# Project-MONAI/GenerativeModels

Measured on NVIDIA H100. Metric: ddim50_voxels_per_s, higher is better.
Workload: dtype fp16

## Files before the change

generativemodels_b200/csrc/flash_attn.cu:

```cuda
#include "common.cuh"
#include "wgmma.cuh"
#include <cuda.h>
#include <cudaTypedefs.h>
#include <mutex>
#include <string.h>

namespace b200 {

struct FlashDev {
  alignas(64) CUtensorMap tmQ;
  alignas(64) CUtensorMap tmK;
  alignas(64) CUtensorMap tmVt;
  int B, T, S, heads, dh, d_chunks;
  int q_tiles, q_tiles_grid, n_items, n_kv;
  float scale_log2;
  h16* out;
  long long out_bstride, out_pitch;
  const h16* res;
  long long res_bstride, res_pitch;
};

namespace fa {

static constexpr int kThreads = 128;
static constexpr int kBM = 64, kBKV = 64;
static constexpr int kChunkBytes = 64 * 64 * 2;

__device__ __forceinline__ uint32_t smem_u32(const void* p) {
  return static_cast<uint32_t>(__cvta_generic_to_shared(p));
}
__device__ __forceinline__ void mbar_init(uint32_t bar, uint32_t count) {
  asm volatile("mbarrier.init.shared::cta.b64 [%0], %1;" ::"r"(bar), "r"(count));
}
__device__ __forceinline__ void mbar_expect_tx(uint32_t bar, uint32_t bytes) {
  asm volatile("mbarrier.arrive.expect_tx.shared::cta.b64 _, [%0], %1;" ::"r"(bar), "r"(bytes) : "memory");
}
__device__ __forceinline__ void mbar_wait(uint32_t bar, uint32_t parity) {
  uint32_t done;
  do {
    asm volatile(
        "{\n\t.reg .pred p;\n\t"
        "mbarrier.try_wait.parity.shared::cta.b64 p, [%1], %2;\n\t"
        "selp.u32 %0, 1, 0, p;\n\t}"
        : "=r"(done)
        : "r"(bar), "r"(parity)
        : "memory");
  } while (!done);
}
__device__ __forceinline__ void mbar_arrive_cluster(uint32_t bar, uint32_t cta) {
  uint32_t remote;
  asm volatile("mapa.shared::cluster.u32 %0, %1, %2;" : "=r"(remote) : "r"(bar), "r"(cta));
  asm volatile("mbarrier.arrive.shared::cluster.b64 _, [%0];" ::"r"(remote) : "memory");
}
__device__ __forceinline__ void tma_load_3d(const CUtensorMap* tm, uint32_t bar, uint32_t dst, int c0, int c1, int c2) {
  asm volatile(
      "cp.async.bulk.tensor.3d.shared::cluster.global.mbarrier::complete_tx::bytes"
      " [%0], [%1, {%3, %4, %5}], [%2];" ::"r"(dst),
      "l"(reinterpret_cast<uint64_t>(tm)), "r"(bar), "r"(c0), "r"(c1), "r"(c2)
      : "memory");
}
__device__ __forceinline__ void tma_load_3d_multicast(const CUtensorMap* tm, uint32_t bar, uint32_t dst, int c0, int c1,
                                                      int c2, uint16_t cta_mask) {
  asm volatile(
      "cp.async.bulk.tensor.3d.shared::cluster.global.mbarrier::complete_tx::bytes.multicast::cluster"
      " [%0], [%1, {%3, %4, %5}], [%2], %6;" ::"r"(dst),
      "l"(reinterpret_cast<uint64_t>(tm)), "r"(bar), "r"(c0), "r"(c1), "r"(c2), "h"(cta_mask)
      : "memory");
}
__device__ __forceinline__ uint32_t cluster_ctarank() {
  uint32_t r;
  asm volatile("mov.u32 %0, %%cluster_ctarank;" : "=r"(r));
  return r;
}
__device__ __forceinline__ void cluster_sync() {
  asm volatile("barrier.cluster.arrive.release.aligned;\n\tbarrier.cluster.wait.acquire.aligned;" ::: "memory");
}
__device__ __forceinline__ void named_sync(uint32_t id, uint32_t threads) {
  asm volatile("bar.sync %0, %1;" ::"r"(id), "r"(threads) : "memory");
}
__device__ __forceinline__ float ex2_approx(float x) {
  float y;
  asm("ex2.approx.ftz.f32 %0, %1;" : "=f"(y) : "f"(x));
  return y;
}
__device__ __forceinline__ uint32_t pack_h2(float lo, float hi) {
  h162 v = f2h2(lo, hi);
  return *reinterpret_cast<uint32_t*>(&v);
}

template <int DCH>
__global__ void __launch_bounds__(kThreads, 1) flash_attn_kernel(const __grid_constant__ FlashDev p) {
  constexpr int DV = 64 * DCH;
  extern __shared__ uint8_t smem_raw[];
  const uint32_t q_base = (smem_u32(smem_raw) + 1023u) & ~1023u;
// ... 11 lines not shown
  const int q0 = qt * kBM;
  const int qc = h * p.dh;
  const int vc = qc;

  pdl_launch_dependents();
  if (tid == 0) {
    mbar_init(q_bar, 1);
    mbar_init(k_bar, 1);
    mbar_init(v_bar, 1);
    asm volatile("fence.mbarrier_init.release.cluster;" ::: "memory");
    asm volatile("fence.proxy.async.shared::cta;" ::: "memory");
  }
  __syncthreads();
  pdl_wait();
  if (tid == 0) {
    mbar_expect_tx(q_bar, DCH * kChunkBytes);
    for (int c = 0; c < DCH; ++c) tma_load_3d(&p.tmQ, q_bar, q_base + c * kChunkBytes, qc + 64 * c, q0, b);
    mbar_expect_tx(k_bar, DCH * kChunkBytes);
    for (int c = 0; c < DCH; ++c) tma_load_3d(&p.tmK, k_bar, k_base + c * kChunkBytes, qc + 64 * c, 0, b);
    mbar_expect_tx(v_bar, DV * kBKV * 2);
    tma_load_3d(&p.tmVt, v_bar, v_base, 0, vc, b);
  }

  float o[DV / 2];
#pragma unroll
  for (int i = 0; i < DV / 2; ++i) o[i] = 0.f;
  float m0 = -INFINITY, m1 = -INFINITY, l0 = 0.f, l1 = 0.f;
  const float sc = p.scale_log2;
  mbar_wait(q_bar, 0);

  for (int j = 0; j < p.n_kv; ++j) {
    const uint32_t ph = j & 1;
    float s[32];
    mbar_wait(k_bar, ph);
    wgmma_fence();
#pragma unroll
    for (int c = 0; c < DCH; ++c) {
      const uint64_t qd = wgmma_desc(q_base + c * kChunkBytes), kd = wgmma_desc(k_base + c * kChunkBytes);
#pragma unroll
      for (int kk = 0; kk < 4; ++kk) wgmma_ss<64>(s, qd + 2u * kk, kd + 2u * kk, (c | kk) != 0 ? 1u : 0u);
    }
    wgmma_commit();
    wgmma_wait<0>();
    wgmma_touch<32>(s);
    __syncthreads();
    if (tid == 0 && j + 1 < p.n_kv) {
      mbar_expect_tx(k_bar, DCH * kChunkBytes);
      for (int c = 0; c < DCH; ++c) tma_load_3d(&p.tmK, k_bar, k_base + c * kChunkBytes, qc + 64 * c, (j + 1) * kBKV, b);
    }

    const int key0 = j * kBKV + 2 * (lane & 3);
    float mx0 = -INFINITY, mx1 = -INFINITY;
#pragma unroll
    for (int n = 0; n < 8; ++n) {
#pragma unroll
      for (int e = 0; e < 2; ++e) {
        const bool ok = key0 + 8 * n + e < p.S;
        s[4 * n + e] = ok ? s[4 * n + e] * sc : -INFINITY;
        s[4 * n + 2 + e] = ok ? s[4 * n + 2 + e] * sc : -INFINITY;
        mx0 = fmaxf(mx0, s[4 * n + e]);
        mx1 = fmaxf(mx1, s[4 * n + 2 + e]);
      }
// ... 24 lines not shown
    for (int n = 0; n < DV / 8; ++n) {
      o[4 * n] *= a0; o[4 * n + 1] *= a0;
      o[4 * n + 2] *= a1; o[4 * n + 3] *= a1;
    }

    mbar_wait(v_bar, ph);
    wgmma_fence();
    const uint64_t vd = wgmma_desc(v_base);
#pragma unroll
    for (int kk = 0; kk < 4; ++kk) wgmma_rs<DV>(o, pa + 4 * kk, vd + 2u * kk, 1u);
    wgmma_commit();
    wgmma_wait<0>();
    wgmma_touch<DV / 2>(o);
    __syncthreads();
    if (tid == 0 && j + 1 < p.n_kv) {
      mbar_expect_tx(v_bar, DV * kBKV * 2);
      tma_load_3d(&p.tmVt, v_bar, v_base, (j + 1) * kBKV, vc, b);
    }
  }

  l0 += __shfl_xor_sync(0xffffffffu, l0, 1);
  l0 += __shfl_xor_sync(0xffffffffu, l0, 2);
  l1 += __shfl_xor_sync(0xffffffffu, l1, 1);
  l1 += __shfl_xor_sync(0xffffffffu, l1, 2);
  const float inv0 = 1.f / l0, inv1 = 1.f / l1;
  const int r0 = 16 * warp + (lane >> 2);
#pragma unroll
  for (int half = 0; half < 2; ++half) {
    const int t = q0 + r0 + 8 * half;
    if (t >= p.T) continue;
    const float inv = half ? inv1 : inv0;
// ... 56 lines not shown
  pdl_launch_dependents();
  if (tid == 0) {
    mbar_init(q_bar, 1);
    for (int s = 0; s < kRing; ++s) {
      mbar_init(full0 + 8 * s, 1);
      mbar_init(empty0 + 8 * s, 4 * kCluster);
    }
    asm volatile("fence.mbarrier_init.release.cluster;" ::: "memory");
  }
  cluster_sync();
  pdl_wait();

  if (wg == 0) {
    setmaxnreg_dec<kProducerRegs>();
    if (tid == 0) {
      mbar_expect_tx(q_bar, 8 * kChunkBytes);
      for (int c = 0; c < 8; ++c) tma_load_3d(&p.tmQ, q_bar, q_base + c * kChunkBytes, qc + 64 * c, q0, b);
      for (int j = 0; j < p.n_kv; ++j) {
        for (int n = 0; n < kChunksPerBlock; ++n) {
          const int slot = n % kRing;
          mbar_wait(empty0 + 8 * slot, ((n / kRing) & 1) ^ 1);
          mbar_expect_tx(full0 + 8 * slot, kChunkBytes);
          if ((n & 1) != (int)rank) continue;
          const uint32_t dst = ring + slot * kChunkBytes, fb = full0 + 8 * slot;
          if (n < 16) {
            const int d = (n & 3) | ((n >> 3) << 2);
            tma_load_3d_multicast(&p.tmK, fb, dst, qc + 64 * d, j * kBlockKeys + 64 * ((n >> 2) & 1), b, 0x3);
          } else {
            const int g = (n - 16) >> 2;
            tma_load_3d_multicast(&p.tmVt, fb, dst, j * kBlockKeys + 64 * (g >> 1), qc + 256 * (g & 1) + 64 * (n & 3), b,
                                  0x3);
          }
        }
      }
    }
  } else {
    setmaxnreg_inc<kConsumerRegs>();
// ... 268 lines not shown
```

generativemodels_b200/csrc/igemm.cu:

```cuda
#include "common.cuh"
#include "wgmma.cuh"
#include <cuda.h>
#include <cudaTypedefs.h>
#include <mutex>
#include <stdlib.h>
#include <string.h>

namespace b200 {

static constexpr int kBM = 128;
static constexpr int kBK = 64;
static constexpr int kABytes = kBM * kBK * 2;
static constexpr int kMmaWarp0 = 4;
static constexpr int kTmaWarp = 12;
static constexpr int kThreads = 13 * 32;

struct SegDev {
  int8_t src, dw, dh, dd;
  uint16_t c0, nchunks;
};

struct IgemmDev {
  alignas(64) CUtensorMap tmA[2];
  alignas(64) CUtensorMap tmB;
// ... 26 lines not shown
  long long out_sN, out_sD, out_sH, out_sW;
  const float* bias;
  const float* rowvec;
  long long rowvec_bstride;
  const float* row_bias;
  int act1, act2;
  int bias_prefetch;
  int geglu;
  float scale;
  const void* res_ptr;
  int res_dtype, res_vec, res_v256;
  long long res_sN, res_sD, res_sH, res_sW;
  SegDev seg[B200_IGEMM_MAX_SEG];
};

__device__ __forceinline__ uint32_t smem_u32(const void* p) {
  return static_cast<uint32_t>(__cvta_generic_to_shared(p));
}
__device__ __forceinline__ void mbar_init(uint32_t bar, uint32_t count) {
  asm volatile("mbarrier.init.shared::cta.b64 [%0], %1;" ::"r"(bar), "r"(count));
}
__device__ __forceinline__ void mbar_arrive_expect_tx(uint32_t bar, uint32_t bytes) {
  asm volatile("mbarrier.arrive.expect_tx.shared::cta.b64 _, [%0], %1;" ::"r"(bar), "r"(bytes) : "memory");
}
__device__ __forceinline__ void mbar_arrive(uint32_t bar) {
  asm volatile("mbarrier.arrive.shared::cta.b64 _, [%0];" ::"r"(bar) : "memory");
}
__device__ __forceinline__ void mbar_wait(uint32_t bar, uint32_t parity) {
  uint32_t done;
  do {
    asm volatile(
        "{\n\t.reg .pred p;\n\t"
        "mbarrier.try_wait.parity.shared::cta.b64 p, [%1], %2;\n\t"
        "selp.u32 %0, 1, 0, p;\n\t}"
        : "=r"(done)
        : "r"(bar), "r"(parity)
        : "memory");
  } while (!done);
}
__device__ __forceinline__ void mbar_wait_warp(uint32_t bar, uint32_t parity) {
  if ((threadIdx.x & 31) == 0) mbar_wait(bar, parity);
  __syncwarp();
}
__device__ __forceinline__ void tma_load_5d(const CUtensorMap* tm, uint32_t bar, uint32_t dst, int c0,
                                            int c1, int c2, int c3, int c4) {
  asm volatile(
      "cp.async.bulk.tensor.5d.shared::cluster.global.mbarrier::complete_tx::bytes"
      " [%0], [%1, {%3, %4, %5, %6, %7}], [%2];" ::"r"(dst),
      "l"(reinterpret_cast<uint64_t>(tm)), "r"(bar), "r"(c0), "r"(c1), "r"(c2), "r"(c3), "r"(c4)
      : "memory");
}
__device__ __forceinline__ void tma_load_3d(const CUtensorMap* tm, uint32_t bar, uint32_t dst, int c0,
                                            int c1, int c2) {
  asm volatile(
      "cp.async.bulk.tensor.3d.shared::cluster.global.mbarrier::complete_tx::bytes"
      " [%0], [%1, {%3, %4, %5}], [%2];" ::"r"(dst),
      "l"(reinterpret_cast<uint64_t>(tm)), "r"(bar), "r"(c0), "r"(c1), "r"(c2)
      : "memory");
}
template <int CH>
__device__ __forceinline__ void acc_ld(const float* src, uint32_t* r) {
#pragma unroll
  for (int j = 0; j < CH; j += 4) {
    const float4 t = *reinterpret_cast<const float4*>(src + j);
    r[j] = __float_as_uint(t.x); r[j + 1] = __float_as_uint(t.y);
    r[j + 2] = __float_as_uint(t.z); r[j + 3] = __float_as_uint(t.w);
  }
}

__host__ __device__ __forceinline__ int split_begin(int num_k, int splits, int ks) {
  return (int)(((long long)num_k * ks) / splits);
}

template <int CH>
// ... 153 lines not shown
    }
  }
  act_inplace<CH>(v, p.act2);
  if (p.out_dtype == B200_DT_H16) {
    h16* o = reinterpret_cast<h16*>(p.out_ptr) + out_off + col0;
    uint4 pk[CH / 8];
#pragma unroll
    for (int g = 0; g < CH / 8; ++g) pk[g] = pack8(v + g * 8);
    if (p.out_v256) {
#pragma unroll
      for (int g = 0; g < CH / 16; ++g) stg256(o + g * 16, pk[2 * g], pk[2 * g + 1]);
    } else {
#pragma unroll
      for (int g = 0; g < CH / 8; ++g) *reinterpret_cast<uint4*>(o + g * 8) = pk[g];
    }
    if constexpr (CH == 32) {
      if (gs) {
        if (p.gn_sh == 3) {
#pragma unroll
          for (int g = 0; g < 4; ++g) {
            float f[8];
            unpack8(pk[g], f);
#pragma unroll
            for (int j = 0; j < 8; ++j) { gs[g] += f[j]; gs[4 + g] = fmaf(f[j], f[j], gs[4 + g]); }
          }
        } else {
#pragma unroll
          for (int g = 0; g < 4; ++g) {
            float f[8];
            unpack8(pk[g], f);
#pragma unroll
            for (int j = 0; j < 8; ++j) {
              gs[2 * g + (j >> 2)] += f[j];
              gs[8 + 2 * g + (j >> 2)] = fmaf(f[j], f[j], gs[8 + 2 * g + (j >> 2)]);
            }
          }
        }
      }
    }
  } else {
    float* o = reinterpret_cast<float*>(p.out_ptr) + out_off + col0;
#pragma unroll
    for (int g = 0; g < CH / 4; ++g)
      *reinterpret_cast<float4*>(o + g * 4) = make_float4(v[g * 4], v[g * 4 + 1], v[g * 4 + 2], v[g * 4 + 3]);
  }
}

template <int CH>
__device__ __forceinline__ void epilogue_row(const IgemmDev& p, float* v, int nb, int ow, long long out_off,
                                             long long res_off, int col0) {
// ... 540 lines not shown
      if (want_key >= 0) {
#pragma unroll
        for (int i = 0; i < PER; ++i)
          if (lane + 32 * i < BN) addv_other[lane + 32 * i] = nbv[i] + nrw[i];
        next_key = want_key;
      }
      __syncwarp();
      if (lane == 0) mbar_arrive(tempty_bar);
    }
    if (gn_on) { __syncwarp(); gn_flush(); }
  }

  __syncthreads();
}

__global__ void igemm_check_kernel(const __grid_constant__ IgemmDev p) {
  pdl_entry();
  const long long rows = (long long)p.N * p.OD * p.OH * p.OW;
  const int col_groups = (p.out_cols + 15) / 16;
  const long long idx = (long long)blockIdx.x * blockDim.x + threadIdx.x;
  if (idx >= rows * col_groups) return;
  const int cg = (int)(idx % col_groups);
  long long m = idx / col_groups;
  const int ow = (int)(m % p.OW); m /= p.OW;
  const int oh = (int)(m % p.OH); m /= p.OH;
  const int od = (int)(m % p.OD); m /= p.OD;
  const int nb = (int)m;
  float acc[16];
#pragma unroll
  for (int j = 0; j < 16; ++j) acc[j] = 0.f;
// ... 145 lines not shown
    v[0] += a.x; v[1] += a.y; v[2] += a.z; v[3] += a.w;
    v[4] += b.x; v[5] += b.y; v[6] += b.z; v[7] += b.w;
  }
  const long long out_off = nb * p.out_sN + od * p.out_sD + oh * p.out_sH + ow * p.out_sW;
  const long long res_off = nb * p.res_sN + od * p.res_sD + oh * p.res_sH + ow * p.res_sW;
  epilogue_math<8>(p, v, nb, ow, res_off, col0);
  store_direct<8>(p, v, out_off, col0);
}

struct Plan {
  TileShape ts;
  long long m_tiles, ntiles, rows;
  int kchunks, BN, tiles_n;
  int splits, ws_cols;
  long long ws_bytes;
};
static int env_int(const char* name, int dflt) {
  const char* e = getenv(name);
  return (e && *e) ? atoi(e) : dflt;
}
static int narrow_min_chunks() { static int v = env_int("B200_NARROW_MIN_CHUNKS", 4); return v; }
static int bias_prefetch_mode() { static int v = env_int("B200_BIAS_PREFETCH", 1); return v; }
static int no_v256() { static int v = env_int("B200_NO_V256", 0); return v; }
static int narrow_one_wave() { static int v = env_int("B200_NARROW_ONE_WAVE", 1); return v; }
static int split_min() { static int v = env_int("B200_SPLIT_MIN", 3); return v; }
static int split_range_min() { static int v = env_int("B200_SPLIT_RANGE_MIN", 32); return v < 1 ? 1 : v; }
static Plan make_plan(const b200_igemm_params* p, bool allow_split, int nsm = 0) {
  if (nsm <= 0) nsm = sm_count();
  Plan pl;
  pl.kchunks = 0;
  for (int s = 0; s < p->n_seg; ++s) pl.kchunks += p->seg[s].nchunks;
  pl.ts = choose_tile(p->out_W, p->out_H, p->out_D, p->stride_w, p->stride_h, p->stride_d);
  const long long tw = (p->out_W + pl.ts.bw - 1) / pl.ts.bw, th = (p->out_H + pl.ts.bh - 1) / pl.ts.bh,
                  td = (p->out_D + pl.ts.bd - 1) / pl.ts.bd;
  pl.m_tiles = tw * th * td * p->out_N;
  pl.rows = (long long)p->out_N * p->out_D * p->out_H * p->out_W;
  pl.splits = 1;
  pl.ws_cols = ((p->out_cols + 7) / 8) * 8;
  pl.ws_bytes = 0;
  const int cols16 = (((p->act1 == B200_ACT_GEGLU ? p->cout : p->out_cols) + 15) / 16) * 16;
  int BN = cols16 <= 16 ? 16 : cols16 <= 32 ? 32 : cols16 <= 64 ? 64 : 128;
  if (p->stat_ptr) BN = 128;
  const long long wide_tiles = pl.m_tiles * ((cols16 + BN - 1) / BN);
  if (allow_split && !p->stat_ptr && !p->gn_partial && p->impl != 1 && p->act1 != B200_ACT_GEGLU && pl.kchunks >= 16 &&
      wide_tiles * 2 <= nsm) {
    long long s = nsm / wide_tiles;
    if (s > pl.kchunks / split_range_min()) s = pl.kchunks / split_range_min();
    if (s > 32) s = 32;
    if (s >= split_min()) {
      pl.splits = (int)s;
      pl.ws_bytes = s * pl.rows * pl.ws_cols * 4;
    }
  }
  if (pl.splits == 1) {
// ... 16 lines not shown
  constexpr int kStageBytes = kABytes + BN * kBK * 2;
  constexpr int smem = 1024 + STAGES * kStageBytes + kBM * (BN + 4) * 4 + 256 + 4 * 32 * 33 * 4 + 8 * BN * 4;
  static_assert(smem <= 227 * 1024, "igemm: shared memory over the 227 KB a block may use");
  static std::once_flag attr_once;
  static cudaError_t attr_rc = cudaSuccess;
  std::call_once(attr_once, [] {
    attr_rc = cudaFuncSetAttribute(igemm_tc_kernel<BN, STAGES>, cudaFuncAttributeMaxDynamicSharedMemorySize, smem);
  });
  B200_CUDA(attr_rc);
  const int grid = d.num_tiles < sm_count() ? d.num_tiles : sm_count();
  B200_CUDA(b200::launch_pdl(igemm_tc_kernel<BN, STAGES>, grid, kThreads, smem, stream, d));
  B200_LAUNCH_CHECK("igemm_tc_kernel");
  return B200_OK;
}

static int env_impl() {
  static int v = -1;
  if (v < 0) {
    const char* e = getenv("B200_IGEMM_IMPL");
    v = (e && strcmp(e, "check") == 0) ? 1 : 0;
  }
  return v;
}

}

using namespace b200;

extern "C" int64_t b200_igemm_split_workspace_bytes(const b200_igemm_params* p) {
  if (!p || p->n_seg < 1 || p->n_seg > B200_IGEMM_MAX_SEG || p->out_N < 1 || p->out_D < 1 || p->out_H < 1 ||
      p->out_W < 1 || p->out_cols < 1 || p->stride_d < 1 || p->stride_h < 1 || p->stride_w < 1)
    return 0;
  if ((p->impl ? p->impl : env_impl()) == 1) return 0;
  return make_plan(p, true).ws_bytes;
}

extern "C" int b200_igemm_plan(const b200_igemm_params* p, int32_t sm_count_, int32_t with_workspace, int32_t out[4]) {
// ... 98 lines not shown
  d.stat_ptr = p->stat_ptr;
  if (p->stat_ptr)
    B200_CHECK_ARG(p->out_N == 1 && p->out_D == 1 && p->out_H == 1, "igemm: stat_ptr needs a GEMM-shaped call");
  if (p->res_ptr) {
    const int g = (p->res_dtype == B200_DT_H16) ? 8 : 4;
    d.res_vec = (p->out_cols % g == 0) && (p->res_sN % g == 0) && (p->res_sD % g == 0) &&
                (p->res_sH % g == 0) && (p->res_sW % g == 0) && (((uintptr_t)p->res_ptr) % 16 == 0);
    d.res_v256 = d.res_vec && p->res_dtype == B200_DT_H16 && (p->out_cols % 16 == 0) && (p->res_sN % 16 == 0) &&
                 (p->res_sD % 16 == 0) && (p->res_sH % 16 == 0) && (p->res_sW % 16 == 0) &&
                 (((uintptr_t)p->res_ptr) % 32 == 0);
    B200_CHECK_ARG(!p->gn_partial || (d.res_vec && p->res_dtype == B200_DT_H16),
                   "igemm: gn_partial needs a vector-aligned h16 residual");
  }

  const int impl = p->impl ? p->impl : env_impl();
  if (impl == 1) {
    const long long rows = (long long)d.N * d.OD * d.OH * d.OW;
    const long long total = rows * ((d.out_cols + 15) / 16);
    const int threads = 128;
    const long long blocks = (total + threads - 1) / threads;
    B200_CHECK_ARG(blocks < (1ll << 31), "igemm(check): problem too large");
    B200_CUDA(b200::launch_pdl(igemm_check_kernel, (unsigned)blocks, threads, 0, stream, d));
    B200_LAUNCH_CHECK("igemm_check_kernel");
    if (d.gn_partial) {
      const long long tot = rows * (d.cout >> d.gn_sh);
      B200_CUDA(b200::launch_pdl(gn8_partial_check_kernel, (unsigned)((tot + 255) / 256), 256, 0, stream, d));
      B200_LAUNCH_CHECK("gn8_partial_check_kernel");
    }
    return B200_OK;
  }
// ... 34 lines not shown
                          CU_TENSOR_MAP_SWIZZLE_128B, CU_TENSOR_MAP_L2_PROMOTION_L2_256B,
                          CU_TENSOR_MAP_FLOAT_OOB_FILL_NONE);
    if (r != CUDA_SUCCESS) {
      set_error("igemm: cuTensorMapEncodeTiled(A%d) failed with %d (C=%d pitch=%d in=%dx%dx%dx%d box=%ux%ux%u)",
                s, (int)r, p->a_C[s], p->a_pitch[s], p->in_N, p->in_D, p->in_H, p->in_W, box[1], box[2], box[3]);
      return B200_ECUDA;
    }
  }
  if (!p->a_ptr[1]) d.tmA[1] = d.tmA[0];
  {
    const int wbn = p->w_batched ? p->in_N : 1;
    cuuint64_t dims[3] = {(cuuint64_t)w_K, (cuuint64_t)p->w_rows, (cuuint64_t)wbn};
    cuuint64_t bs = p->w_bstride ? (cuuint64_t)p->w_bstride * 2 : (cuuint64_t)p->w_rows * p->w_pitch * 2;
    cuuint64_t strides[2] = {(cuuint64_t)p->w_pitch * 2, bs};
    B200_CHECK_ARG(bs % 16 == 0, "igemm: weight batch stride not 16-byte aligned");
    cuuint32_t box[3] = {(cuuint32_t)kBK, (cuuint32_t)BN, 1};
    cuuint32_t estr[3] = {1, 1, 1};
    CUresult r = g_encode(&d.tmB, B200_H16_TMAP, 3, const_cast<void*>(p->w_ptr), dims,
                          strides, box, estr, CU_TENSOR_MAP_INTERLEAVE_NONE, CU_TENSOR_MAP_SWIZZLE_128B,
                          CU_TENSOR_MAP_L2_PROMOTION_L2_256B, CU_TENSOR_MAP_FLOAT_OOB_FILL_NONE);
    if (r != CUDA_SUCCESS) {
      set_error("igemm: cuTensorMapEncodeTiled(W) failed with %d (K=%d rows=%d pitch=%d)", (int)r, w_K,
                p->w_rows, p->w_pitch);
      return B200_ECUDA;
    }
  }

  auto launch = [&](const IgemmDev& dev) {
    switch (BN) {
      case 16:  return launch_tc<16, 8>(dev, stream);
      case 32:  return launch_tc<32, 8>(dev, stream);
      case 64:  return launch_tc<64, 6>(dev, stream);
      default:  return launch_tc<128, 4>(dev, stream);
    }
  };
  if (splits == 1) return launch(d);

  if (p->split_counters) {
    B200_CHECK_ARG(pl.ntiles <= B200_IGEMM_SPLIT_COUNTERS, "igemm: %lld output tiles exceed the %d split-K tickets",
                   pl.ntiles, B200_IGEMM_SPLIT_COUNTERS);
    IgemmDev df = d;
    df.k_splits = splits;
// ... 30 lines not shown
```

generativemodels_b200/csrc/wgmma.cuh:

```cuda
#pragma once
#include "common.cuh"

#ifdef B200_H16_IS_BF16
#define B200_WGMMA_AB "bf16"
#else
#define B200_WGMMA_AB "f16"
#endif

namespace b200 {

__device__ __forceinline__ uint64_t wgmma_desc(uint32_t smem_addr) {
  uint64_t d = 0;
  d |= static_cast<uint64_t>((smem_addr & 0x3FFFFu) >> 4);
  d |= static_cast<uint64_t>(1) << 16;
  d |= static_cast<uint64_t>(1024 >> 4) << 32;
  d |= static_cast<uint64_t>(1) << 62;
  return d;
}
__device__ __forceinline__ void wgmma_fence() { asm volatile("wgmma.fence.sync.aligned;" ::: "memory"); }
__device__ __forceinline__ void wgmma_commit() { asm volatile("wgmma.commit_group.sync.aligned;" ::: "memory"); }
template <int N>
__device__ __forceinline__ void wgmma_wait() { asm volatile("wgmma.wait_group.sync.aligned %0;" ::"n"(N) : "memory"); }
template <int R>
__device__ __forceinline__ void wgmma_touch(float* d) {
// ... 96 lines not shown
      "{\n\t.reg .pred p;\n\t"
      "setp.ne.b32 p, %133, 0;\n\t"
      "wgmma.mma_async.sync.aligned.m64n256k16.f32." B200_WGMMA_AB "." B200_WGMMA_AB " "
      "{%0, %1, %2, %3, %4, %5, %6, %7, %8, %9, %10, %11, %12, %13, %14, %15, %16, %17, %18, %19, %20, %21, %22, %23, %24, %25, %26, %27, %28, %29, %30, %31, %32, %33, %34, %35, %36, %37, %38, %39, %40, %41, %42, %43, %44, %45, %46, %47, %48, %49, %50, %51, %52, %53, %54, %55, %56, %57, %58, %59, %60, %61, %62, %63, %64, %65, %66, %67, %68, %69, %70, %71, %72, %73, %74, %75, %76, %77, %78, %79, %80, %81, %82, %83, %84, %85, %86, %87, %88, %89, %90, %91, %92, %93, %94, %95, %96, %97, %98, %99, %100, %101, %102, %103, %104, %105, %106, %107, %108, %109, %110, %111, %112, %113, %114, %115, %116, %117, %118, %119, %120, %121, %122, %123, %124, %125, %126, %127}, {%128, %129, %130, %131}, %132, p, 1, 1, 0;\n\t}"
      : "+f"(d[0]), "+f"(d[1]), "+f"(d[2]), "+f"(d[3]), "+f"(d[4]), "+f"(d[5]), "+f"(d[6]), "+f"(d[7]), "+f"(d[8]), "+f"(d[9]), "+f"(d[10]), "+f"(d[11]), "+f"(d[12]), "+f"(d[13]), "+f"(d[14]), "+f"(d[15]), "+f"(d[16]), "+f"(d[17]), "+f"(d[18]), "+f"(d[19]), "+f"(d[20]), "+f"(d[21]), "+f"(d[22]), "+f"(d[23]), "+f"(d[24]), "+f"(d[25]), "+f"(d[26]), "+f"(d[27]), "+f"(d[28]), "+f"(d[29]), "+f"(d[30]), "+f"(d[31]), "+f"(d[32]), "+f"(d[33]), "+f"(d[34]), "+f"(d[35]), "+f"(d[36]), "+f"(d[37]), "+f"(d[38]), "+f"(d[39]), "+f"(d[40]), "+f"(d[41]), "+f"(d[42]), "+f"(d[43]), "+f"(d[44]), "+f"(d[45]), "+f"(d[46]), "+f"(d[47]), "+f"(d[48]), "+f"(d[49]), "+f"(d[50]), "+f"(d[51]), "+f"(d[52]), "+f"(d[53]), "+f"(d[54]), "+f"(d[55]), "+f"(d[56]), "+f"(d[57]), "+f"(d[58]), "+f"(d[59]), "+f"(d[60]), "+f"(d[61]), "+f"(d[62]), "+f"(d[63]), "+f"(d[64]), "+f"(d[65]), "+f"(d[66]), "+f"(d[67]), "+f"(d[68]), "+f"(d[69]), "+f"(d[70]), "+f"(d[71]), "+f"(d[72]), "+f"(d[73]), "+f"(d[74]), "+f"(d[75]), "+f"(d[76]), "+f"(d[77]), "+f"(d[78]), "+f"(d[79]), "+f"(d[80]), "+f"(d[81]), "+f"(d[82]), "+f"(d[83]), "+f"(d[84]), "+f"(d[85]), "+f"(d[86]), "+f"(d[87]), "+f"(d[88]), "+f"(d[89]), "+f"(d[90]), "+f"(d[91]), "+f"(d[92]), "+f"(d[93]), "+f"(d[94]), "+f"(d[95]), "+f"(d[96]), "+f"(d[97]), "+f"(d[98]), "+f"(d[99]), "+f"(d[100]), "+f"(d[101]), "+f"(d[102]), "+f"(d[103]), "+f"(d[104]), "+f"(d[105]), "+f"(d[106]), "+f"(d[107]), "+f"(d[108]), "+f"(d[109]), "+f"(d[110]), "+f"(d[111]), "+f"(d[112]), "+f"(d[113]), "+f"(d[114]), "+f"(d[115]), "+f"(d[116]), "+f"(d[117]), "+f"(d[118]), "+f"(d[119]), "+f"(d[120]), "+f"(d[121]), "+f"(d[122]), "+f"(d[123]), "+f"(d[124]), "+f"(d[125]), "+f"(d[126]), "+f"(d[127])
      : "r"(a[0]), "r"(a[1]), "r"(a[2]), "r"(a[3]), "l"(bdesc), "r"(accumulate));
}

template <int N>
__device__ __forceinline__ void wgmma_rs(float* d, const uint32_t* a, uint64_t bdesc, uint32_t accumulate) {
  if constexpr (N == 64) wgmma_rs_n64(d, a, bdesc, accumulate);
  else if constexpr (N == 128) wgmma_rs_n128(d, a, bdesc, accumulate);
  else wgmma_rs_n256(d, a, bdesc, accumulate);
}

}
```

Before: 87530.

## Add 2-CTA cluster 128x256 warp-specialized implicit GEMM with multicast weight tiles

Adds a new implicit-GEMM kernel for wide convolutions. It uses 256-column output tiles, a 2-CTA cluster that multicasts weight halves through TMA, a 4-stage mbarrier ring, and one producer warpgroup feeding two consumer warpgroups. The fused epilogue covers bias, residual and group-norm partial statistics. The kernel is picked automatically for large multi-segment convolutions whose cout is a multiple of 256. It aims to raise operand reuse and tensor-core utilisation, at the cost of register pressure, cluster scheduling constraints and a more complex epilogue. Shared mbarrier/TMA helpers move into a common header and the group-norm accumulation is generalised to any CH.

```diff
diff --git a/generativemodels_b200/csrc/flash_attn.cu b/generativemodels_b200/csrc/flash_attn.cu
--- a/generativemodels_b200/csrc/flash_attn.cu
+++ b/generativemodels_b200/csrc/flash_attn.cu
@@ -26,58 +26,6 @@
 static constexpr int kBM = 64, kBKV = 64;
 static constexpr int kChunkBytes = 64 * 64 * 2;
 
-__device__ __forceinline__ uint32_t smem_u32(const void* p) {
-  return static_cast<uint32_t>(__cvta_generic_to_shared(p));
-}
-__device__ __forceinline__ void mbar_init(uint32_t bar, uint32_t count) {
-  asm volatile("mbarrier.init.shared::cta.b64 [%0], %1;" ::"r"(bar), "r"(count));
-}
-__device__ __forceinline__ void mbar_expect_tx(uint32_t bar, uint32_t bytes) {
-  asm volatile("mbarrier.arrive.expect_tx.shared::cta.b64 _, [%0], %1;" ::"r"(bar), "r"(bytes) : "memory");
-}
-__device__ __forceinline__ void mbar_wait(uint32_t bar, uint32_t parity) {
-  uint32_t done;
-  do {
-    asm volatile(
-        "{\n\t.reg .pred p;\n\t"
-        "mbarrier.try_wait.parity.shared::cta.b64 p, [%1], %2;\n\t"
-        "selp.u32 %0, 1, 0, p;\n\t}"
-        : "=r"(done)
-        : "r"(bar), "r"(parity)
-        : "memory");
-  } while (!done);
-}
-__device__ __forceinline__ void mbar_arrive_cluster(uint32_t bar, uint32_t cta) {
-  uint32_t remote;
-  asm volatile("mapa.shared::cluster.u32 %0, %1, %2;" : "=r"(remote) : "r"(bar), "r"(cta));
-  asm volatile("mbarrier.arrive.shared::cluster.b64 _, [%0];" ::"r"(remote) : "memory");
-}
-__device__ __forceinline__ void tma_load_3d(const CUtensorMap* tm, uint32_t bar, uint32_t dst, int c0, int c1, int c2) {
-  asm volatile(
-      "cp.async.bulk.tensor.3d.shared::cluster.global.mbarrier::complete_tx::bytes"
-      " [%0], [%1, {%3, %4, %5}], [%2];" ::"r"(dst),
-      "l"(reinterpret_cast<uint64_t>(tm)), "r"(bar), "r"(c0), "r"(c1), "r"(c2)
-      : "memory");
-}
-__device__ __forceinline__ void tma_load_3d_multicast(const CUtensorMap* tm, uint32_t bar, uint32_t dst, int c0, int c1,
-                                                      int c2, uint16_t cta_mask) {
-  asm volatile(
-      "cp.async.bulk.tensor.3d.shared::cluster.global.mbarrier::complete_tx::bytes.multicast::cluster"
-      " [%0], [%1, {%3, %4, %5}], [%2], %6;" ::"r"(dst),
-      "l"(reinterpret_cast<uint64_t>(tm)), "r"(bar), "r"(c0), "r"(c1), "r"(c2), "h"(cta_mask)
-      : "memory");
-}
-__device__ __forceinline__ uint32_t cluster_ctarank() {
-  uint32_t r;
-  asm volatile("mov.u32 %0, %%cluster_ctarank;" : "=r"(r));
-  return r;
-}
-__device__ __forceinline__ void cluster_sync() {
-  asm volatile("barrier.cluster.arrive.release.aligned;\n\tbarrier.cluster.wait.acquire.aligned;" ::: "memory");
-}
-__device__ __forceinline__ void named_sync(uint32_t id, uint32_t threads) {
-  asm volatile("bar.sync %0, %1;" ::"r"(id), "r"(threads) : "memory");
-}
 __device__ __forceinline__ float ex2_approx(float x) {
   float y;
   asm("ex2.approx.ftz.f32 %0, %1;" : "=f"(y) : "f"(x));
@@ -119,11 +67,11 @@
   __syncthreads();
   pdl_wait();
   if (tid == 0) {
-    mbar_expect_tx(q_bar, DCH * kChunkBytes);
+    mbar_arrive_expect_tx(q_bar, DCH * kChunkBytes);
     for (int c = 0; c < DCH; ++c) tma_load_3d(&p.tmQ, q_bar, q_base + c * kChunkBytes, qc + 64 * c, q0, b);
-    mbar_expect_tx(k_bar, DCH * kChunkBytes);
+    mbar_arrive_expect_tx(k_bar, DCH * kChunkBytes);
     for (int c = 0; c < DCH; ++c) tma_load_3d(&p.tmK, k_bar, k_base + c * kChunkBytes, qc + 64 * c, 0, b);
-    mbar_expect_tx(v_bar, DV * kBKV * 2);
+    mbar_arrive_expect_tx(v_bar, DV * kBKV * 2);
     tma_load_3d(&p.tmVt, v_bar, v_base, 0, vc, b);
   }
 
@@ -150,7 +98,7 @@
     wgmma_touch<32>(s);
     __syncthreads();
     if (tid == 0 && j + 1 < p.n_kv) {
-      mbar_expect_tx(k_bar, DCH * kChunkBytes);
+      mbar_arrive_expect_tx(k_bar, DCH * kChunkBytes);
       for (int c = 0; c < DCH; ++c) tma_load_3d(&p.tmK, k_bar, k_base + c * kChunkBytes, qc + 64 * c, (j + 1) * kBKV, b);
     }
 
@@ -205,7 +153,7 @@
     wgmma_touch<DV / 2>(o);
     __syncthreads();
     if (tid == 0 && j + 1 < p.n_kv) {
-      mbar_expect_tx(v_bar, DV * kBKV * 2);
+      mbar_arrive_expect_tx(v_bar, DV * kBKV * 2);
       tma_load_3d(&p.tmVt, v_bar, v_base, (j + 1) * kBKV, vc, b);
     }
   }
@@ -292,13 +240,13 @@
   if (wg == 0) {
     setmaxnreg_dec<kProducerRegs>();
     if (tid == 0) {
-      mbar_expect_tx(q_bar, 8 * kChunkBytes);
+      mbar_arrive_expect_tx(q_bar, 8 * kChunkBytes);
       for (int c = 0; c < 8; ++c) tma_load_3d(&p.tmQ, q_bar, q_base + c * kChunkBytes, qc + 64 * c, q0, b);
       for (int j = 0; j < p.n_kv; ++j) {
         for (int n = 0; n < kChunksPerBlock; ++n) {
           const int slot = n % kRing;
           mbar_wait(empty0 + 8 * slot, ((n / kRing) & 1) ^ 1);
-          mbar_expect_tx(full0 + 8 * slot, kChunkBytes);
+          mbar_arrive_expect_tx(full0 + 8 * slot, kChunkBytes);
           if ((n & 1) != (int)rank) continue;
           const uint32_t dst = ring + slot * kChunkBytes, fb = full0 + 8 * slot;
           if (n < 16) {
diff --git a/generativemodels_b200/csrc/igemm.cu b/generativemodels_b200/csrc/igemm.cu
--- a/generativemodels_b200/csrc/igemm.cu
+++ b/generativemodels_b200/csrc/igemm.cu
@@ -64,34 +64,6 @@
   SegDev seg[B200_IGEMM_MAX_SEG];
 };
 
-__device__ __forceinline__ uint32_t smem_u32(const void* p) {
-  return static_cast<uint32_t>(__cvta_generic_to_shared(p));
-}
-__device__ __forceinline__ void mbar_init(uint32_t bar, uint32_t count) {
-  asm volatile("mbarrier.init.shared::cta.b64 [%0], %1;" ::"r"(bar), "r"(count));
-}
-__device__ __forceinline__ void mbar_arrive_expect_tx(uint32_t bar, uint32_t bytes) {
-  asm volatile("mbarrier.arrive.expect_tx.shared::cta.b64 _, [%0], %1;" ::"r"(bar), "r"(bytes) : "memory");
-}
-__device__ __forceinline__ void mbar_arrive(uint32_t bar) {
-  asm volatile("mbarrier.arrive.shared::cta.b64 _, [%0];" ::"r"(bar) : "memory");
-}
-__device__ __forceinline__ void mbar_wait(uint32_t bar, uint32_t parity) {
-  uint32_t done;
-  do {
-    asm volatile(
-        "{\n\t.reg .pred p;\n\t"
-        "mbarrier.try_wait.parity.shared::cta.b64 p, [%1], %2;\n\t"
-        "selp.u32 %0, 1, 0, p;\n\t}"
-        : "=r"(done)
-        : "r"(bar), "r"(parity)
-        : "memory");
-  } while (!done);
-}
-__device__ __forceinline__ void mbar_wait_warp(uint32_t bar, uint32_t parity) {
-  if ((threadIdx.x & 31) == 0) mbar_wait(bar, parity);
-  __syncwarp();
-}
 __device__ __forceinline__ void tma_load_5d(const CUtensorMap* tm, uint32_t bar, uint32_t dst, int c0,
                                             int c1, int c2, int c3, int c4) {
   asm volatile(
@@ -100,14 +72,6 @@
       "l"(reinterpret_cast<uint64_t>(tm)), "r"(bar), "r"(c0), "r"(c1), "r"(c2), "r"(c3), "r"(c4)
       : "memory");
 }
-__device__ __forceinline__ void tma_load_3d(const CUtensorMap* tm, uint32_t bar, uint32_t dst, int c0,
-                                            int c1, int c2) {
-  asm volatile(
-      "cp.async.bulk.tensor.3d.shared::cluster.global.mbarrier::complete_tx::bytes"
-      " [%0], [%1, {%3, %4, %5}], [%2];" ::"r"(dst),
-      "l"(reinterpret_cast<uint64_t>(tm)), "r"(bar), "r"(c0), "r"(c1), "r"(c2)
-      : "memory");
-}
 template <int CH>
 __device__ __forceinline__ void acc_ld(const float* src, uint32_t* r) {
 #pragma unroll
@@ -291,26 +255,25 @@
 #pragma unroll
       for (int g = 0; g < CH / 8; ++g) *reinterpret_cast<uint4*>(o + g * 8) = pk[g];
     }
-    if constexpr (CH == 32) {
-      if (gs) {
-        if (p.gn_sh == 3) {
-#pragma unroll
-          for (int g = 0; g < 4; ++g) {
-            float f[8];
-            unpack8(pk[g], f);
-#pragma unroll
-            for (int j = 0; j < 8; ++j) { gs[g] += f[j]; gs[4 + g] = fmaf(f[j], f[j], gs[4 + g]); }
-          }
-        } else {
-#pragma unroll
-          for (int g = 0; g < 4; ++g) {
-            float f[8];
-            unpack8(pk[g], f);
-#pragma unroll
-            for (int j = 0; j < 8; ++j) {
-              gs[2 * g + (j >> 2)] += f[j];
-              gs[8 + 2 * g + (j >> 2)] = fmaf(f[j], f[j], gs[8 + 2 * g + (j >> 2)]);
-            }
+    if (gs) {
+      constexpr int G8 = CH / 8, G4 = CH / 4;
+      if (p.gn_sh == 3) {
+#pragma unroll
+        for (int g = 0; g < G8; ++g) {
+          float f[8];
+          unpack8(pk[g], f);
+#pragma unroll
+          for (int j = 0; j < 8; ++j) { gs[g] += f[j]; gs[G8 + g] = fmaf(f[j], f[j], gs[G8 + g]); }
+        }
+      } else {
+#pragma unroll
+        for (int g = 0; g < G8; ++g) {
+          float f[8];
+          unpack8(pk[g], f);
+#pragma unroll
+          for (int j = 0; j < 8; ++j) {
+            gs[2 * g + (j >> 2)] += f[j];
+            gs[G4 + 2 * g + (j >> 2)] = fmaf(f[j], f[j], gs[G4 + 2 * g + (j >> 2)]);
           }
         }
       }
@@ -881,6 +844,226 @@
   __syncthreads();
 }
 
+namespace wide {
+static constexpr int kThreads = 384;
+static constexpr int kCluster = 2;
+static constexpr int kBN = 256;
+static constexpr int kStages = 4;
+static constexpr int kBHalfBytes = 128 * kBK * 2;
+static constexpr int kStageBytes = kABytes + 2 * kBHalfBytes;
+static constexpr int kSliceLd = 36;
+static constexpr int kOffSlice = kStages * kStageBytes;
+static constexpr int kOffAdd = kOffSlice + 8 * 16 * kSliceLd * 4;
+static constexpr int kOffBar = kOffAdd + 8 * kBN * 4;
+static constexpr int kSmem = 1024 + kOffBar + 2 * kStages * 8;
+static constexpr int kProducerRegs = 40, kConsumerRegs = 232;
+static_assert(kProducerRegs * 128 + kConsumerRegs * 256 <= 65536, "register budget of one CTA per SM");
+}
+
+__device__ __forceinline__ float gn_reduce16(const float* gs, int lane, int gn_sh) {
+  const bool h3 = (lane & 8) != 0, h2 = (lane & 4) != 0, h1 = (lane & 2) != 0;
+  if (gn_sh == 3) {
+    float a[2];
+#pragma unroll
+    for (int i = 0; i < 2; ++i) a[i] = (h3 ? gs[2 + i] : gs[i]) + __shfl_xor_sync(0xffffffffu, h3 ? gs[i] : gs[2 + i], 8);
+    float c = (h2 ? a[1] : a[0]) + __shfl_xor_sync(0xffffffffu, h2 ? a[0] : a[1], 4);
+    c += __shfl_xor_sync(0xffffffffu, c, 2);
+    c += __shfl_xor_sync(0xffffffffu, c, 1);
+    return c;
+  }
+  float a4[4], a2[2];
+#pragma unroll
+  for (int i = 0; i < 4; ++i) a4[i] = (h3 ? gs[4 + i] : gs[i]) + __shfl_xor_sync(0xffffffffu, h3 ? gs[i] : gs[4 + i], 8);
+#pragma unroll
+  for (int i = 0; i < 2; ++i) a2[i] = (h2 ? a4[2 + i] : a4[i]) + __shfl_xor_sync(0xffffffffu, h2 ? a4[i] : a4[2 + i], 4);
+  float c = (h1 ? a2[1] : a2[0]) + __shfl_xor_sync(0xffffffffu, h1 ? a2[0] : a2[1], 2);
+  c += __shfl_xor_sync(0xffffffffu, c, 1);
+  return c;
+}
+
+__global__ void __launch_bounds__(wide::kThreads, 1) igemm_wide_kernel(const __grid_constant__ IgemmDev p) {
+  using namespace wide;
+  if (!p.pdl_late) pdl_launch_dependents();
+  extern __shared__ uint8_t smem_raw[];
+  uint8_t* sm = smem_raw + ((1024u - (smem_u32(smem_raw) & 1023u)) & 1023u);
+  const uint32_t ring = smem_u32(sm);
+  const uint32_t full0 = ring + kOffBar, empty0 = full0 + 8 * kStages;
+
+  const int tid = threadIdx.x;
+  const int wg = __shfl_sync(0xffffffffu, tid >> 7, 0);
+  const uint32_t rank = cluster_ctarank();
+  const int cid = (int)blockIdx.x / kCluster, n_clusters = (int)gridDim.x / kCluster;
+  const int m_tiles = p.tiles_w * p.tiles_h * p.tiles_d * p.N;
+  const int num_units = p.num_tiles;
+  const int num_k = p.num_k_chunks;
+
+  if (tid == 0) {
+    for (int s = 0; s < kStages; ++s) {
+      mbar_init(full0 + 8 * s, 1);
+      mbar_init(empty0 + 8 * s, 8 * kCluster);
+    }
+    asm volatile("fence.mbarrier_init.release.cluster;" ::: "memory");
+  }
+  cluster_sync();
+  pdl_wait();
+
+  struct MTile { int nt, wt, ht, dt, nb; bool ok; };
+  auto unit_tile = [&](int u) {
+    MTile t;
+    t.nt = u % p.tiles_n;
+    int m = 2 * (u / p.tiles_n) + (int)rank;
+    t.ok = m < m_tiles;
+    if (!t.ok) m = m_tiles - 1;
+    t.wt = m % p.tiles_w; m /= p.tiles_w;
+    t.ht = m % p.tiles_h; m /= p.tiles_h;
+    t.dt = m % p.tiles_d;
+    t.nb = m / p.tiles_d;
+    return t;
+  };
+
+  if (wg == 0) {
+    setmaxnreg_dec<kProducerRegs>();
+    if (tid == 0) {
+      int stage = 0;
+      uint32_t phase = 0;
+      for (int u = cid; u < num_units; u += n_clusters) {
+        const MTile t = unit_tile(u);
+        const int iw0 = t.wt * p.BW * p.sw, ih0 = t.ht * p.BH * p.sh, id0 = t.dt * p.BD * p.sd;
+        const int wrow = t.nt * kBN + 128 * (int)rank;
+        int kglob = 0;
+        for (int s = 0; s < p.n_seg; ++s) {
+          const SegDev sg = p.seg[s];
+          const CUtensorMap* tm = &p.tmA[sg.src];
+          const int cw = iw0 + sg.dw, ch = ih0 + sg.dh, cd = id0 + sg.dd;
+          for (int c = 0; c < sg.nchunks; ++c, ++kglob) {
+            mbar_wait(empty0 + 8 * stage, phase ^ 1u);
+            const uint32_t dst = ring + stage * kStageBytes, fb = full0 + 8 * stage;
+            mbar_arrive_expect_tx(fb, kStageBytes);
+            tma_load_5d(tm, fb, dst, (sg.c0 + c) * kBK, cw, ch, cd, t.nb);
+            tma_load_3d_multicast(&p.tmB, fb, dst + kABytes + rank * kBHalfBytes, kglob * kBK, wrow, 0, 0x3);
+            if (++stage == kStages) { stage = 0; phase ^= 1u; }
+          }
+        }
+      }
+      if (p.pdl_late) pdl_launch_dependents();
+    }
+  } else {
+    setmaxnreg_inc<kConsumerRegs>();
+    const int c = wg - 1;
+    const int wq = (tid >> 5) & 3;
+    const int lane = tid & 31;
+    float* slice = reinterpret_cast<float*>(sm + kOffSlice) + (4 * c + wq) * 16 * kSliceLd;
+    float* addv = reinterpret_cast<float*>(sm + kOffAdd) + (4 * c + wq) * kBN;
+    const int er = 64 * c + 16 * wq + (lane & 15);
+    const int eh = lane >> 4;
+    const int rw = er & (p.BW - 1), rh = (er >> p.bw_log2) & (p.BH - 1), rd = er >> (p.bw_log2 + p.bh_log2);
+    auto release = [&](int s) {
+      __syncwarp();
+      if (lane == 0) {
+        mbar_arrive_cluster(empty0 + 8 * s, 0);
+        mbar_arrive_cluster(empty0 + 8 * s, 1);
+      }
+    };
+
+    const bool gn_on = p.gn_partial != nullptr;
+    const int gsh = p.gn_sh;
+    float gacc[kBN / 32];
+#pragma unroll
+    for (int s = 0; s < kBN / 32; ++s) gacc[s] = 0.f;
+    int key = -1, gn_nb = 0, gn_n0 = 0;
+    auto gn_flush = [&]() {
+      const bool writer = (lane & (gsh == 3 ? 3 : 1)) == 0;
+      const int stat = (lane >> 3) & 1;
+      const int gl = gsh == 3 ? (lane >> 2) & 1 : ((lane >> 1) & 3);
+      float* dst = p.gn_partial +
+                   (((long long)gn_nb * p.gn_slots + p.gn_slot0 + 4 * blockIdx.x + wq) * (p.cout >> gsh)) * 2 + stat;
+      for (int pass = 0; pass < 2; ++pass) {
+        if (pass == c && writer) {
+#pragma unroll
+          for (int s = 0; s < kBN / 32; ++s) dst[(((gn_n0 + 32 * s + 16 * eh) >> gsh) + gl) * 2] += gacc[s];
+        }
+        if (pass == 0) named_sync(1, 256);
+      }
+#pragma unroll
+      for (int s = 0; s < kBN / 32; ++s) gacc[s] = 0.f;
+    };
+
+    float acc[kBN / 2];
+    int stage = 0;
+    uint32_t phase = 0;
+    for (int u = cid; u < num_units; u += n_clusters) {
+      int prev = -1;
+      for (int k = 0; k < num_k; ++k) {
+        mbar_wait(full0 + 8 * stage, phase);
+        const uint32_t st = ring + stage * kStageBytes;
+        const uint64_t adesc = wgmma_desc(st + c * (64 * kBK * 2));
+        const uint64_t bdesc = wgmma_desc(st + kABytes);
+        wgmma_fence();
+#pragma unroll
+        for (int kk = 0; kk < kBK / 16; ++kk)
+          wgmma_ss<kBN>(acc, adesc + 2u * kk, bdesc + 2u * kk, (k | kk) != 0 ? 1u : 0u);
+        wgmma_commit();
+        wgmma_wait<1>();
+        if (prev >= 0) release(prev);
+        prev = stage;
+        if (++stage == kStages) { stage = 0; phase ^= 1u; }
+      }
+      wgmma_wait<0>();
+      wgmma_touch<kBN / 2>(acc);
+      release(prev);
+
+      const MTile t = unit_tile(u);
+      const int n0 = t.nt * kBN;
+      const int ow = t.wt * p.BW + rw, oh = t.ht * p.BH + rh, od = t.dt * p.BD + rd;
+      const bool row_ok = t.ok && ow < p.OW && oh < p.OH && od < p.OD;
+      const long long out_off = t.nb * p.out_sN + od * p.out_sD + oh * p.out_sH + ow * p.out_sW;
+      const long long res_off = t.nb * p.res_sN + od * p.res_sD + oh * p.res_sH + ow * p.res_sW;
+      if (t.nb * p.tiles_n + t.nt != key) {
+        if (gn_on && key >= 0) gn_flush();
+        key = t.nb * p.tiles_n + t.nt;
+        gn_nb = t.nb;
+        gn_n0 = n0;
+        float bv[kBN / 32], rv[kBN / 32];
+#pragma unroll
+        for (int i = 0; i < kBN / 32; ++i) {
+          const int col = n0 + lane + 32 * i;
+          bv[i] = p.bias ? __ldg(p.bias + col) : 0.f;
+          rv[i] = p.rowvec ? __ldg(p.rowvec + (long long)t.nb * p.rowvec_bstride + col) : 0.f;
+        }
+        __syncwarp();
+#pragma unroll
+        for (int i = 0; i < kBN / 32; ++i) addv[lane + 32 * i] = bv[i] + rv[i];
+        __syncwarp();
+      }
+      const bool res_on = p.res_ptr && row_ok;
+      uint4 rv_next[2] = {make_uint4(0u, 0u, 0u, 0u), make_uint4(0u, 0u, 0u, 0u)};
+      if (res_on) load_res_fast<16>(p, rv_next, res_off, n0 + 16 * eh);
+#pragma unroll
+      for (int s = 0; s < kBN / 32; ++s) {
+        __syncwarp();
+#pragma unroll
+        for (int j = 4 * s; j < 4 * s + 4; ++j) {
+          const int col = 8 * (j - 4 * s) + 2 * (lane & 3);
+          *reinterpret_cast<float2*>(slice + (lane >> 2) * kSliceLd + col) = make_float2(acc[4 * j], acc[4 * j + 1]);
+          *reinterpret_cast<float2*>(slice + ((lane >> 2) + 8) * kSliceLd + col) =
+              make_float2(acc[4 * j + 2], acc[4 * j + 3]);
+        }
+        __syncwarp();
+        uint32_t raw[16];
+        acc_ld<16>(slice + (lane & 15) * kSliceLd + 16 * eh, raw);
+        const uint4 rv[2] = {rv_next[0], rv_next[1]};
+        if (res_on && s + 1 < kBN / 32) load_res_fast<16>(p, rv_next, res_off, n0 + 32 * (s + 1) + 16 * eh);
+        const int cc = 32 * s + 16 * eh;
+        float gs[8] = {0.f, 0.f, 0.f, 0.f, 0.f, 0.f, 0.f, 0.f};
+        if (row_ok) epilogue_fast<16>(p, raw, addv + cc, rv, out_off, n0 + cc, gs);
+        if (gn_on) gacc[s] += gn_reduce16(gs, lane, gsh);
+      }
+    }
+    if (gn_on && key >= 0) gn_flush();
+  }
+  cluster_sync();
+}
+
 __global__ void igemm_check_kernel(const __grid_constant__ IgemmDev p) {
   pdl_entry();
   const long long rows = (long long)p.N * p.OD * p.OH * p.OW;
@@ -1056,7 +1239,27 @@
   int kchunks, BN, tiles_n;
   int splits, ws_cols;
   long long ws_bytes;
+  bool wide;
 };
+
+static int env_impl() {
+  static int v = -1;
+  if (v < 0) {
+    const char* e = getenv("B200_IGEMM_IMPL");
+    v = (e && strcmp(e, "check") == 0) ? 1 : 0;
+  }
+  return v;
+}
+
+static bool wide_fits(const b200_igemm_params* p) {
+  auto v8 = [](long long a, long long b, long long c, long long d) { return a % 8 == 0 && b % 8 == 0 && c % 8 == 0 && d % 8 == 0; };
+  const bool out_vec = v8(p->out_sN, p->out_sD, p->out_sH, p->out_sW) && ((uintptr_t)p->out_ptr % 16) == 0;
+  const bool res_ok = !p->res_ptr || (p->res_dtype == B200_DT_H16 && v8(p->res_sN, p->res_sD, p->res_sH, p->res_sW) &&
+                                      ((uintptr_t)p->res_ptr % 16) == 0);
+  return p->out_dtype == B200_DT_H16 && p->cout == p->out_cols && p->cout % wide::kBN == 0 && out_vec && res_ok &&
+         !p->stat_ptr && p->act1 != B200_ACT_GEGLU && !p->row_bias && !p->w_batched && !p->a_broadcast;
+}
+static constexpr int kWideMinChunks = 32;
 static int env_int(const char* name, int dflt) {
   const char* e = getenv(name);
   return (e && *e) ? atoi(e) : dflt;
@@ -1080,6 +1283,15 @@
   pl.splits = 1;
   pl.ws_cols = ((p->out_cols + 7) / 8) * 8;
   pl.ws_bytes = 0;
+  const int impl = p->impl ? p->impl : env_impl();
+  pl.wide = wide_fits(p) && (impl == 3 || (impl == 0 && p->n_seg >= 8 && pl.kchunks >= kWideMinChunks &&
+                                            ((pl.m_tiles + 1) / 2) * (p->cout / wide::kBN) >= nsm / wide::kCluster));
+  if (pl.wide) {
+    pl.BN = wide::kBN;
+    pl.tiles_n = p->cout / wide::kBN;
+    pl.ntiles = ((pl.m_tiles + 1) / 2) * pl.tiles_n;
+    return pl;
+  }
   const int cols16 = (((p->act1 == B200_ACT_GEGLU ? p->cout : p->out_cols) + 15) / 16) * 16;
   int BN = cols16 <= 16 ? 16 : cols16 <= 32 ? 32 : cols16 <= 64 ? 64 : 128;
   if (p->stat_ptr) BN = 128;
@@ -1126,13 +1338,34 @@
   return B200_OK;
 }
 
-static int env_impl() {
-  static int v = -1;
-  if (v < 0) {
-    const char* e = getenv("B200_IGEMM_IMPL");
-    v = (e && strcmp(e, "check") == 0) ? 1 : 0;
-  }
-  return v;
+static int launch_wide(const IgemmDev& d, cudaStream_t stream) {
+  static_assert(wide::kSmem <= 227 * 1024, "igemm: shared memory over the 227 KB a block may use");
+  static std::once_flag once;
+  static cudaError_t rc = cudaSuccess;
+  static int max_clusters = 0;
+  std::call_once(once, [] {
+    rc = cudaFuncSetAttribute(igemm_wide_kernel, cudaFuncAttributeMaxDynamicSharedMemorySize, wide::kSmem);
+    if (rc != cudaSuccess) return;
+    cudaLaunchConfig_t cfg = {};
+    cfg.gridDim = dim3(wide::kCluster);
+    cfg.blockDim = dim3(wide::kThreads);
+    cfg.dynamicSmemBytes = wide::kSmem;
+    cudaLaunchAttribute attr;
+    attr.id = cudaLaunchAttributeClusterDimension;
+    attr.val.clusterDim.x = wide::kCluster;
+    attr.val.clusterDim.y = 1;
+    attr.val.clusterDim.z = 1;
+    cfg.attrs = &attr;
+    cfg.numAttrs = 1;
+    rc = cudaOccupancyMaxActiveClusters(&max_clusters, igemm_wide_kernel, &cfg);
+  });
+  B200_CUDA(rc);
+  if (max_clusters < 1) { set_error("igemm: no cluster of igemm_wide_kernel fits on this device"); return B200_ECUDA; }
+  const int clusters = d.num_tiles < max_clusters ? d.num_tiles : max_clusters;
+  B200_CUDA(b200::launch_cluster(igemm_wide_kernel, wide::kCluster, clusters * wide::kCluster, wide::kThreads,
+                                 wide::kSmem, stream, d));
+  B200_LAUNCH_CHECK("igemm_wide_kernel");
+  return B200_OK;
 }
 
 }
@@ -1261,6 +1494,11 @@
   }
 
   const int impl = p->impl ? p->impl : env_impl();
+  B200_CHECK_ARG(impl >= 0 && impl <= 3, "igemm: impl %d not in 0..3", impl);
+  B200_CHECK_ARG(impl != 3 || wide_fits(p),
+                 "igemm: impl 3 (128 x 256 tiles) needs a vector-aligned h16 output with cout == out_cols a multiple of "
+                 "256, a vector-aligned h16 residual or none, and no stat_ptr / GEGLU / row_bias / batched weights / "
+                 "broadcast A");
   if (impl == 1) {
     const long long rows = (long long)d.N * d.OD * d.OH * d.OW;
     const long long total = rows * ((d.out_cols + 15) / 16);
@@ -1325,7 +1563,7 @@
     cuuint64_t bs = p->w_bstride ? (cuuint64_t)p->w_bstride * 2 : (cuuint64_t)p->w_rows * p->w_pitch * 2;
     cuuint64_t strides[2] = {(cuuint64_t)p->w_pitch * 2, bs};
     B200_CHECK_ARG(bs % 16 == 0, "igemm: weight batch stride not 16-byte aligned");
-    cuuint32_t box[3] = {(cuuint32_t)kBK, (cuuint32_t)BN, 1};
+    cuuint32_t box[3] = {(cuuint32_t)kBK, (cuuint32_t)(pl.wide ? 128 : BN), 1};
     cuuint32_t estr[3] = {1, 1, 1};
     CUresult r = g_encode(&d.tmB, B200_H16_TMAP, 3, const_cast<void*>(p->w_ptr), dims,
                           strides, box, estr, CU_TENSOR_MAP_INTERLEAVE_NONE, CU_TENSOR_MAP_SWIZZLE_128B,
@@ -1337,6 +1575,7 @@
     }
   }
 
+  if (pl.wide) return launch_wide(d, stream);
   auto launch = [&](const IgemmDev& dev) {
     switch (BN) {
       case 16:  return launch_tc<16, 8>(dev, stream);
diff --git a/generativemodels_b200/csrc/wgmma.cuh b/generativemodels_b200/csrc/wgmma.cuh
--- a/generativemodels_b200/csrc/wgmma.cuh
+++ b/generativemodels_b200/csrc/wgmma.cuh
@@ -1,5 +1,6 @@
 #pragma once
 #include "common.cuh"
+#include <cuda.h>
 
 #ifdef B200_H16_IS_BF16
 #define B200_WGMMA_AB "bf16"
@@ -134,4 +135,60 @@
   else wgmma_rs_n256(d, a, bdesc, accumulate);
 }
 
+__device__ __forceinline__ uint32_t smem_u32(const void* p) {
+  return static_cast<uint32_t>(__cvta_generic_to_shared(p));
 }
+__device__ __forceinline__ void mbar_init(uint32_t bar, uint32_t count) {
+  asm volatile("mbarrier.init.shared::cta.b64 [%0], %1;" ::"r"(bar), "r"(count));
+}
+__device__ __forceinline__ void mbar_arrive_expect_tx(uint32_t bar, uint32_t bytes) {
+  asm volatile("mbarrier.arrive.expect_tx.shared::cta.b64 _, [%0], %1;" ::"r"(bar), "r"(bytes) : "memory");
+}
+__device__ __forceinline__ void mbar_arrive(uint32_t bar) {
+  asm volatile("mbarrier.arrive.shared::cta.b64 _, [%0];" ::"r"(bar) : "memory");
+}
+__device__ __forceinline__ void mbar_wait(uint32_t bar, uint32_t parity) {
+  uint32_t done;
+  do {
+    asm volatile(
+        "{\n\t.reg .pred p;\n\t"
+        "mbarrier.try_wait.parity.shared::cta.b64 p, [%1], %2;\n\t"
+        "selp.u32 %0, 1, 0, p;\n\t}"
+        : "=r"(done)
+        : "r"(bar), "r"(parity)
+        : "memory");
+  } while (!done);
+}
+__device__ __forceinline__ void mbar_arrive_cluster(uint32_t bar, uint32_t cta) {
+  uint32_t remote;
+  asm volatile("mapa.shared::cluster.u32 %0, %1, %2;" : "=r"(remote) : "r"(bar), "r"(cta));
+  asm volatile("mbarrier.arrive.shared::cluster.b64 _, [%0];" ::"r"(remote) : "memory");
+}
+__device__ __forceinline__ void tma_load_3d(const CUtensorMap* tm, uint32_t bar, uint32_t dst, int c0, int c1, int c2) {
+  asm volatile(
+      "cp.async.bulk.tensor.3d.shared::cluster.global.mbarrier::complete_tx::bytes"
+      " [%0], [%1, {%3, %4, %5}], [%2];" ::"r"(dst),
+      "l"(reinterpret_cast<uint64_t>(tm)), "r"(bar), "r"(c0), "r"(c1), "r"(c2)
+      : "memory");
+}
+__device__ __forceinline__ void tma_load_3d_multicast(const CUtensorMap* tm, uint32_t bar, uint32_t dst, int c0, int c1,
+                                                      int c2, uint16_t cta_mask) {
+  asm volatile(
+      "cp.async.bulk.tensor.3d.shared::cluster.global.mbarrier::complete_tx::bytes.multicast::cluster"
+      " [%0], [%1, {%3, %4, %5}], [%2], %6;" ::"r"(dst),
+      "l"(reinterpret_cast<uint64_t>(tm)), "r"(bar), "r"(c0), "r"(c1), "r"(c2), "h"(cta_mask)
+      : "memory");
+}
+__device__ __forceinline__ uint32_t cluster_ctarank() {
+  uint32_t r;
+  asm volatile("mov.u32 %0, %%cluster_ctarank;" : "=r"(r));
+  return r;
+}
+__device__ __forceinline__ void cluster_sync() {
+  asm volatile("barrier.cluster.arrive.release.aligned;\n\tbarrier.cluster.wait.acquire.aligned;" ::: "memory");
+}
+__device__ __forceinline__ void named_sync(uint32_t id, uint32_t threads) {
+  asm volatile("bar.sync %0, %1;" ::"r"(id), "r"(threads) : "memory");
+}
+
+}
```

Result: faster. 106,000, median of 6 (+21.1%).
